# angelvillar96/STLPose

Hardware: AMD Instinct MI355X
Metric: images/sec/GPU HRNet-W32 384x288 train step; PCKh@0.5 parity (higher is better)
Workload: dtype f16/bf16; 1 GPU; HRNet-W32 384x288 bs=32/GPU train step (fwd+MSE+bwd+Adam), random-init weights; global_batch=32, parallelism=dp1

## Files before the change

### include/stlpose_hip.h

```cpp
#ifndef STLPOSE_HIP_H
#define STLPOSE_HIP_H
#include <stdint.h>
#ifdef __cplusplus
extern "C" {
#endif

#define STL_F32 0
#define STL_BF16 1
#define STL_F16 2
#define STL_NSHARD 2

#define STL_DT2(grad_dtype, fwd_dtype) ((grad_dtype) | ((fwd_dtype) << 8))

#define STL_SRC_PLAIN 0
#define STL_SRC_BN 1
#define STL_SRC_BNBWD 2
#define STL_SRC_BNADD 3

typedef struct stl_src {
    const void* x;
    const void* y;
    int32_t mode;
    int32_t relu;
    const double* stats;
// ... 16 lines not shown
    stl_src src;
    const void* w;
    void* out;
    const float* bias;
    int32_t out_relu;
    double* out_stats;
    const void* addend;
    const void* mask_y;
    stl_src mask_bn;
    double* red;
    const void* mask_z;
    void* src_out;
    int32_t ydtype, pad_;
} stl_conv;
int stl_conv_forward(const stl_conv* p, void* stream);
int stl_conv_plan(stl_conv* p);
int stl_conv_bnadd_ok(const stl_conv* p);

typedef struct stl_wgrad {
    int32_t dtype;
    int32_t B, Hi, Wi, Ci, Ho, Wo, Co, ks, stride;
    int32_t TH, TW, nsplit;
    stl_src h;
    stl_src g;
    float* partial;
    int32_t ydtype;
} stl_wgrad;
int stl_conv_wgrad(const stl_wgrad* p, void* stream);
#define STL_WGRAD_GROUP_MAX 8
typedef struct stl_wgrad_io { stl_src h; stl_src g; float* partial; } stl_wgrad_io;
typedef struct stl_wgrad_group { int32_t n, pad_; const stl_wgrad* p[STL_WGRAD_GROUP_MAX]; } stl_wgrad_group;
int stl_conv_wgrad_group(const stl_wgrad_group* g, void* stream);
int stl_wgrad_chunk(const stl_wgrad* p);

typedef struct stl_term {
    stl_src src;
    int32_t shift;
} stl_term;
typedef struct stl_fuse {
    int32_t dtype, B, H, W, C, nterms, relu;
    stl_term t[4];
    void* out;
} stl_fuse;
int stl_fuse_forward(const stl_fuse* p, void* stream);

typedef struct stl_fuse_bwd {
    int32_t dtype, B, H, W, C, ngrads, relu, nbn;
    const void* dz[4];
    const void* z;
    void* du;
    stl_src bn[4];
    double* rstats[4];
    int32_t ydtype, pad_;
} stl_fuse_bwd;
int stl_fuse_backward(const stl_fuse_bwd* p, void* stream);

typedef struct stl_upbwd {
    int32_t dtype, B, H, W, C, shift;
    const void* du;
    void* dt;
    stl_src bn;
    double* rstats;
    int32_t ydtype, pad_;
} stl_upbwd;
int stl_upsample_backward(const stl_upbwd* p, void* stream);

// ... 301 lines not shown
```

### stlpose_amd/build.py

```python
from __future__ import annotations

import glob
import hashlib
import os
import subprocess
import sys
from concurrent.futures import ThreadPoolExecutor

HERE = os.path.dirname(os.path.abspath(__file__))
CSRC = os.path.join(HERE, "csrc")
INCLUDE = os.path.join(HERE, "..", "include")
LIB = os.path.join(HERE, "libstlpose_hip.so")
UNITS = [("capi.hip", "capi", []), ("conv_core.hip", "conv_core_bf16", ["-DSTL_DT=1"]), ("conv_core.hip", "conv_core_f32", ["-DSTL_DT=0"]),
         ("conv_core.hip", "conv_core_f16", ["-DSTL_DT=3"]),
         ("wgrad.hip", "wgrad_bf16", ["-DSTL_DT=1"]), ("wgrad.hip", "wgrad_f32", ["-DSTL_DT=0"]), ("elementwise.hip", "elementwise", []),
         ("program.hip", "program", []), ("retrieval.hip", "retrieval", []),
         ("topdown.hip", "topdown", []), ("detector.hip", "detector", []), ("detector_train.hip", "detector_train", []),
         ("adain.hip", "adain", []), ("box_ap.hip", "box_ap", [])]
HIPCC = os.environ.get("HIPCC", "/opt/rocm/bin/hipcc")
FLAGS = ["--offload-arch=gfx950", "-O3", "-fPIC", "-std=c++17", "-Wno-unused-result", "-Wno-unused-value"]


def source_files():
    return sorted(glob.glob(os.path.join(CSRC, "*.hip")) + glob.glob(os.path.join(CSRC, "*.inc")) + glob.glob(os.path.join(CSRC, "*.cuh"))
                  + glob.glob(os.path.join(INCLUDE, "*.h")))


def source_id() -> str:
    h = hashlib.sha256()
    for f in source_files():
        h.update(os.path.basename(f).encode() + b"\0")
        h.update(open(f, "rb").read())
    return h.hexdigest()[:16]


def _digest(deps, flags) -> str:
    h = hashlib.sha256(" ".join(flags).encode())
    for f in deps:
        h.update(os.path.basename(f).encode() + b"\0")
        h.update(open(f, "rb").read())
    return h.hexdigest()[:16]


def _load_state(path: str) -> dict:
    try:
        import json
        return json.load(open(path))
    except Exception:
# ... 48 lines not shown
```

### stlpose_amd/capi.py

```python
from __future__ import annotations

import ctypes as C
import os

_HERE = os.path.dirname(os.path.abspath(__file__))
LIB_PATH = os.environ.get("STLPOSE_HIP_LIB") or os.path.join(_HERE, "libstlpose_hip.so")

F32, BF16, F16 = 0, 1, 2


def dt2(grad_dtype: int, fwd_dtype: int) -> int:
    return grad_dtype | ((fwd_dtype if fwd_dtype != grad_dtype else 0) << 8)


POSE_APPROACH = {"all_kpts": 0, "full_body": 1, "upper_body": 2}
POSE_DIM = {"all_kpts": 34, "full_body": 26, "upper_body": 18}
POSE_METHOD = {"euclidean": 0, "cosine": 1, "manhattan": 2, "confidence": 3, "oks": 4, "l2sq": 5, "cos_normalised": 6}
POSE_PEN = {"zero_coord": 0, "none": 1, "mean": 2, "max": 3}
POSE_TOPK_MAX, POSE_RANK_MAX, POSE_RANK_LABELS_MAX, POSE_NSCORES = 1024, 16384, 4, 10
POSE_RANK_ANY_MAX = 1 << 24
BOX_MAX, RESIZE_SRC_MAX, RESIZE_DST_MAX = 4096, 16384, 2048
BOX_AP_THRS, BOX_AP_AREAS, BOX_AP_DETS, BOX_AP_GT_MAX, BOX_AP_SCAN_TILE, BOX_AP_MAXDETS_MAX, BOX_AP_RECS_MAX = 10, 4, 100, 128, 1024, 8, 101
DET_NMS_MAX = 65536
GATHER_COPY, GATHER_UP, GATHER_POOL = 0, 1, 2
# ... 112 lines not shown

class DetTerm(C.Structure):
    _fields_ = [("x", vp), ("mode", i32), ("H", i32), ("W", i32), ("pad_", i32)]


class DetFuse(C.Structure):
    _fields_ = [("B", i32), ("H", i32), ("W", i32), ("C", i32), ("nterms", i32), ("pad_", i32), ("t", DetTerm * 3), ("wparam", vp),
                ("out", vp)]


class Op(C.Structure):
    _fields_ = [("kind", i32), ("stream", i32), ("desc", vp), ("nwait", i32), ("wait", i32 * 8), ("record", i32)]


class ReduceRange(C.Structure):
    _fields_ = [("partials", vp), ("grads", vp), ("tab", vp), ("n", i32), ("blk_base", i32), ("nblocks", i32), ("pad_", i32)]


class BNRange(C.Structure):
    _fields_ = [("rstats", vp), ("grads", vp), ("tab", vp), ("n", i32), ("pad_", i32)]


OP_KIND = {"stl_conv_forward": 0, "stl_conv_wgrad": 1, "stl_fuse_forward": 2, "stl_fuse_backward": 3,
           "stl_upsample_backward": 4, "stl_patch3x3": 5, "stl_head_forward": 6, "stl_head_backward": 7,
           "stl_reduce_slabs_range": 8, "stl_bn_grads_range": 9, "stl_conv_wgrad_group": 10,
           "stl_patch3x3_backward": 13}

SIGNATURES = {
    "stl_conv_forward": [C.POINTER(Conv), vp],
    "stl_conv_plan": [C.POINTER(Conv)],
    "stl_conv_bnadd_ok": [C.POINTER(Conv)],
    "stl_conv_wgrad": [C.POINTER(Wgrad), vp],
    "stl_wgrad_chunk": [C.POINTER(Wgrad)],
    "stl_conv_wgrad_group": [C.POINTER(WgradGroup), vp],
    "stl_fuse_forward": [C.POINTER(Fuse), vp],
    "stl_fuse_backward": [C.POINTER(FuseBwd), vp],
    "stl_upsample_backward": [C.POINTER(UpBwd), vp],
    "stl_patch3x3": [i32, vp, vp, i32, i32, i32, i32, vp, vp, vp],
    "stl_patch3x3_backward": [i32, vp, vp, i32, i32, i32, i32, vp, vp],
    "stl_head_forward": [i32, vp, vp, vp, vp, i32, i32, i32, i32, i32, vp],
    "stl_head_backward": [i32, vp, vp, vp, vp, vp, i32, i32, i32, i32, i32, i32, vp],
    "stl_mse_loss": [vp, vp, vp, vp, vp, i32, vp, i32, i32, i32, f32, vp],
    "stl_gaussian_targets": [vp, vp, vp, vp, i32, i32, i32, i32, f32, f32, f32, vp],
    "stl_heatmap_argmax": [vp, vp, vp, vp, i32, i32, i32, vp],
    "stl_flip_merge": [vp, vp, vp, vp, i32, i32, i32, i32, vp],
    "stl_flip_merge_backward": [vp, vp, vp, vp, i32, i32, i32, i32, vp],
    "stl_final_preds": [vp, vp, vp, vp, vp, i32, i32, i32, i32, vp],
    "stl_weight_prep": [i32, vp, vp, vp, i32, i32, vp],
    "stl_reduce_slabs": [vp, vp, vp, i32, i32, vp],
    "stl_reduce_slabs_range": [C.POINTER(ReduceRange), vp],
    "stl_bn_running_update": [vp, vp, vp, vp, i32, f32, vp, vp],
    "stl_bn_param_grads": [vp, vp, vp, i32, vp],
    "stl_adam_step": [vp, vp, vp, vp, i64, vp, vp, vp, vp],
    "stl_sgd_step": [vp, vp, vp, i64, vp, vp, vp, vp],
    "stl_affine_crop": [vp, vp, vp, vp, vp, vp, i32, i32, i32, vp, vp, vp],
    "stl_maxpool2x2": [i32, vp, vp, i32, i32, i32, i32, vp],
    "stl_l1_partial": [i32, vp, vp, i64, vp, i32, vp],
    "stl_l2_partial": [i32, vp, vp, i64, vp, i32, vp],
    "stl_maxpool2x2_backward": [i32, vp, vp, vp, i32, i32, i32, i32, i32, vp],
    "stl_l2_backward": [i32, vp, vp, vp, i64, vp, i32, vp],
    "stl_bilinear_nchw": [vp, vp, i32, i32, i32, i32, i32, i32, vp],
    "stl_sum_partials": [vp, i32, C.c_double, vp, i32, vp],
    "stl_nchw_to_nhwc": [i32, vp, vp, i32, i32, i32, i32, vp],
    "stl_nhwc_to_nchw": [i32, vp, vp, i32, i32, i32, i32, vp],
    "stl_program_create": [C.POINTER(Op), i32, i32, C.POINTER(vp)],
    "stl_program_run": [vp, C.POINTER(vp)],
# ... 95 lines not shown
```

### stlpose_amd/csrc/wgrad.hip

```cpp
#include <type_traits>
#include "common.cuh"

#ifndef STL_DT
#define STL_DT 2
#endif

constexpr int WG_MAXG = STL_WGRAD_GROUP_MAX;
struct WgK {
    stl_wgrad p;
    stl_wgrad_io io[WG_MAXG];
    int ng;
    int dbg;
    int tiles_c, npt, HR, HC, HP, PI, pad, taps;
    int psg, psh;
    int off_cg, off_ch, off_g, off_h;
    float r_TW, r_HC, r_tc, r_vp, r_PI;
    unsigned long long m_tc, m_vp, m_PI;
    int xmap, units, gy, gz;
};

int stl_wgrad_backend_bf16(bool wide, const WgK& k, dim3 grid, size_t lds, hipStream_t st);
int stl_wgrad_backend_f32(bool wide, const WgK& k, dim3 grid, size_t lds, hipStream_t st);

namespace {

#include "conv_common.inc"

#ifdef STL_STAMPS
#include "../../include/stlpose_hip_debug.h"
__device__ long long g_wstamps[16];
__device__ long long g_wstamps2[64];
#define WSTAMP(i)                                                                                   \
    do {                                                                                            \
        if (k.dbg && blockIdx.x == 0 && blockIdx.y == 0 && blockIdx.z == 0 && threadIdx.x == 0) g_wstamps[i] = wall_clock64(); \
    } while (0)
#define WSTAMP2(i)                                                                                  \
    do {                                                                                            \
        if (k.dbg && blockIdx.x == 0 && blockIdx.y == 0 && blockIdx.z == 0 && threadIdx.x == 0 && (i) < 64) g_wstamps2[i] = wall_clock64(); \
    } while (0)
#else
#define WSTAMP(i) do {} while (0)
#define WSTAMP2(i) do {} while (0)
#endif

__device__ __forceinline__ int mad24_vsv(int a, int b_uniform, int c) {
    int r;
    asm("v_mad_i32_i24 %0, %1, %2, %3" : "=v"(r) : "v"(a), "s"(b_uniform), "v"(c));
    return r;
}

__device__ __forceinline__ int sdiv(int n, unsigned long long m) { return (int)(((unsigned long long)(uint32_t)n * m) >> 32); }


struct WgBlock { int member, bsplit, cy, cz; bool live; };
__device__ __forceinline__ WgBlock wg_block(const WgK& k) {
// ... 563 lines not shown
#pragma unroll
        for (int mt = 0; mt < 2; ++mt)
#pragma unroll
            for (int nt = 0; nt < 2; ++nt) {
                const int co = co0 + wm * 32 + mt * 16 + 4 * g, ci = ci0 + wn * 32 + nt * 16 + (lane & 15);
                float* dst = slab + (size_t)co * TAPS * p.Ci + ci;
                const bool ciok = ci < p.Ci;
#pragma unroll
                for (int tap = 0; tap < TAPS; ++tap)
#pragma unroll
                    for (int r = 0; r < 4; ++r)
                        if (ciok && co + r < p.Co) dst[((size_t)r * TAPS + tap) * p.Ci] = acc[mt][nt][tap][r];
            }
    }
    WSTAMP(8);
}

template <typename T, typename TY, int KS, int NVH, bool GQ, int TPX>
int launch64(const WgK& k, dim3 grid, size_t lds, hipStream_t st) {
    static bool attr_done = false;
    if (!attr_done) {
        (void)hipFuncSetAttribute(reinterpret_cast<const void*>(&wgrad64_kernel<T, KS, NVH, GQ, TPX, TY>),
                                  hipFuncAttributeMaxDynamicSharedMemorySize, 160 * 1024);
        attr_done = true;
    }
    STL_LAUNCH((wgrad64_kernel<T, KS, NVH, GQ, TPX, TY>), grid, dim3(256), lds, st, k);
    static char nbuf[160];
    static const char* nm = stl_kname<T>(nbuf, "wgrad64_kernel", {KS, NVH, GQ, TPX, stl_code<TY>()});
    stl_note_kernel(nm, true);
    STL_LAUNCH_CHECK("conv_wgrad64");
    return 0;
}

#if STL_DT != 0
template <typename TY>
int dispatch64(const WgK& k, dim3 grid, size_t lds, hipStream_t st) {
    const int nvh = ceil_div(k.HP * 8, 256);
    const bool gq = k.p.g.mode == STL_SRC_BNBWD;
    if (k.p.TH * k.p.TW <= 128 && nvh <= 6) return gq ? launch64<__bf16, TY, 1, 6, true, 128>(k, grid, lds, st) : launch64<__bf16, TY, 1, 6, false, 128>(k, grid, lds, st);
    return stl_set_error("wgrad64: halo of %d pixels is too large for a %d-pixel tile", k.HP, k.p.TH * k.p.TW);
}
#endif

dim3 wg_grid(WgK& k, int units, int gy, int gz) {
    const int xcd_env = getenv("STL_WGRAD_XCD") ? atoi(getenv("STL_WGRAD_XCD")) : 1;
    k.units = units, k.gy = gy, k.gz = gz;
    k.xmap = xcd_env && gy * gz > 1;
    if (!k.xmap) return dim3(units, gy, gz);
    return dim3(8 * ceil_div(units, 8) * gy * gz, 1, 1);
}

static bool wgrad_c64_3x3(const stl_wgrad& p) {
    const char* e = getenv("STL_WGRAD_C64");
    return !(e && atoi(e) == 0) && p.dtype == STL_BF16 && p.ks == 3 && p.stride == 1 && p.Co >= 64 && p.Ci >= 64;
}

int wgrad_chunk(const stl_wgrad& p) {
    if (wgrad_c64_3x3(p)) return 64;
    return (p.dtype == STL_BF16 && p.ks == 1 && p.stride == 1 && p.Co >= 64 && p.Ci >= 64) ? 64 : 32;
}

template <typename T, typename TY, int KS>
int dispatch(const WgK& k, dim3 grid, size_t lds, hipStream_t st) {
    {
        const int64_t gpx = (int64_t)k.p.B * k.p.Ho * k.p.Wo, hpx = (int64_t)k.p.B * k.p.Hi * k.p.Wi;
        const bool small = gpx * k.p.Co * (int64_t)sizeof(T) < ((int64_t)1 << 32) && hpx * k.p.Ci * (int64_t)sizeof(T) < ((int64_t)1 << 32) &&
                           (int64_t)k.p.Wo * k.p.Co * (int64_t)sizeof(T) < (1 << 23) &&
                           (int64_t)(k.PI > k.p.Hi ? k.PI - k.p.Hi : k.p.Hi - k.PI) * k.p.Wi * k.p.Ci * (int64_t)sizeof(T) < (1 << 23) &&
                           k.PI < (1 << 12) && k.tiles_c < (1 << 12) && (int64_t)k.npt * k.p.TH * k.p.stride < (1 << 20);
        STL_CHECK(small, "wgrad: tensors of 4 GB or more, rows beyond 8 MB or more than 4095 rows / tile columns are not addressable");
    }
    const int vpx = 32 / ET<T>::KV;
    const int nvh = ceil_div(k.HP * vpx, 256);
    const bool gq = k.p.g.mode == STL_SRC_BNBWD;
    STL_CHECK(k.p.TH * k.p.TW <= 128, "wgrad: tiles of more than 128 pixels are not supported");
    if constexpr (KS == 3 && sizeof(T) == 2) {
        if (k.p.ks == 3 && wgrad_c64_3x3(k.p)) {
            const int nvh16 = ceil_div(k.HP * 8, 1024);
            if (nvh16 <= 2) return gq ? launch<T, TY, KS, 2, true, 128, 16, 64>(k, grid, lds, st) : launch<T, TY, KS, 2, false, 128, 16, 64>(k, grid, lds, st);
            if (nvh16 <= 3) return gq ? launch<T, TY, KS, 3, true, 128, 16, 64>(k, grid, lds, st) : launch<T, TY, KS, 3, false, 128, 16, 64>(k, grid, lds, st);
            return stl_set_error("wgrad: halo of %d pixels is too large for the 64-channel 3x3 kernel; shrink the tile", k.HP);
        }
    }
    if constexpr (KS == 3) {
        const int nvh8 = ceil_div(k.HP * vpx, 512);
        if (nvh8 <= 2) return gq ? launch<T, TY, KS, 2, true, 128, 8>(k, grid, lds, st) : launch<T, TY, KS, 2, false, 128, 8>(k, grid, lds, st);
        if (nvh8 <= 3) return gq ? launch<T, TY, KS, 3, true, 128, 8>(k, grid, lds, st) : launch<T, TY, KS, 3, false, 128, 8>(k, grid, lds, st);
        if (nvh8 <= 5) return gq ? launch<T, TY, KS, 5, true, 128, 8>(k, grid, lds, st) : launch<T, TY, KS, 5, false, 128, 8>(k, grid, lds, st);
        if (nvh8 <= 9) return gq ? launch<T, TY, KS, 9, true, 128, 8>(k, grid, lds, st) : launch<T, TY, KS, 9, false, 128, 8>(k, grid, lds, st);
        return stl_set_error("wgrad: halo of %d pixels is too large for the 3x3 kernel; shrink the tile", k.HP);
    }
    if (nvh <= 3) return gq ? launch<T, TY, KS, 3, true>(k, grid, lds, st) : launch<T, TY, KS, 3, false>(k, grid, lds, st);
    if (nvh <= 6) return gq ? launch<T, TY, KS, 6, true>(k, grid, lds, st) : launch<T, TY, KS, 6, false>(k, grid, lds, st);
    if (nvh <= 9) return gq ? launch<T, TY, KS, 9, true>(k, grid, lds, st) : launch<T, TY, KS, 9, false>(k, grid, lds, st);
    if (nvh <= 18) return gq ? launch<T, TY, KS, 18, true>(k, grid, lds, st) : launch<T, TY, KS, 18, false>(k, grid, lds, st);
    return stl_set_error("wgrad: halo of %d pixels needs %d staging vectors per thread (max 18); shrink the tile", k.HP, nvh);
}

}

#if STL_DT != 0
int stl_wgrad_backend_bf16(bool wide, const WgK& k, dim3 grid, size_t lds, hipStream_t st) {
    if (k.p.ydtype == STL_F16) {
        if (wide) return dispatch64<f16>(k, grid, lds, st);
        return k.p.ks == 3 ? dispatch<__bf16, f16, 3>(k, grid, lds, st) : dispatch<__bf16, f16, 1>(k, grid, lds, st);
    }
    if (wide) return dispatch64<__bf16>(k, grid, lds, st);
    return k.p.ks == 3 ? dispatch<__bf16, __bf16, 3>(k, grid, lds, st) : dispatch<__bf16, __bf16, 1>(k, grid, lds, st);
}
#endif
#if STL_DT != 1
int stl_wgrad_backend_f32(bool wide, const WgK& k, dim3 grid, size_t lds, hipStream_t st) {
    if (wide) return stl_set_error("wgrad: the 64 x 64-channel variant is bf16 only");
    return k.p.ks == 3 ? dispatch<float, float, 3>(k, grid, lds, st) : dispatch<float, float, 1>(k, grid, lds, st);
}
#endif

#if STL_DT != 0
#ifdef STL_STAMPS
extern "C" int stl_debug_wgrad_stamps2(long long* host64) {
    return hipMemcpyFromSymbol(host64, HIP_SYMBOL(g_wstamps2), 64 * sizeof(long long)) == hipSuccess ? 0 : stl_set_error("stamps: copy failed");
}
extern "C" int stl_debug_wgrad_stamps(long long* host16) {
    return hipMemcpyFromSymbol(host16, HIP_SYMBOL(g_wstamps), 16 * sizeof(long long)) == hipSuccess ? 0 : stl_set_error("stamps: copy failed");
}
#endif

extern "C" int stl_wgrad_chunk(const stl_wgrad* pp) { return wgrad_chunk(*pp); }

static int wgrad_run(const stl_wgrad* const* ps, int ng, void* stream);

extern "C" int stl_conv_wgrad(const stl_wgrad* pp, void* stream) { return wgrad_run(&pp, 1, stream); }

extern "C" int stl_conv_wgrad_group(const stl_wgrad_group* grp, void* stream) {
    STL_CHECK(grp && grp->n >= 1 && grp->n <= WG_MAXG, "wgrad_group: 1..%d members", WG_MAXG);
    const stl_wgrad& a = *grp->p[0];
    for (int i = 1; i < grp->n; ++i) {
        const stl_wgrad& b = *grp->p[i];
        STL_CHECK(b.dtype == a.dtype && b.B == a.B && b.Hi == a.Hi && b.Wi == a.Wi && b.Ci == a.Ci && b.Ho == a.Ho && b.Wo == a.Wo &&
                      b.Co == a.Co && b.ks == a.ks && b.stride == a.stride && b.TH == a.TH && b.TW == a.TW && b.nsplit == a.nsplit &&
                      b.g.mode == a.g.mode,
                  "wgrad_group: member %d differs from member 0 in geometry, tile, nsplit or gradient source mode", i);
    }
    return wgrad_run(grp->p, grp->n, stream);
}

static int wgrad_run(const stl_wgrad* const* ps, int ng, void* stream) {
    const stl_wgrad& p = *ps[0];
  for (int i_ = 0; i_ < ng; ++i_) {
    const stl_wgrad& p = *ps[i_];
    STL_CHECK(p.dtype == STL_F32 || p.dtype == STL_BF16, "wgrad: bad dtype (gradients are fp32 or bf16)");
    STL_CHECK(p.ydtype == 0 || p.ydtype == p.dtype || (p.dtype == STL_BF16 && p.ydtype == STL_F16), "wgrad: ydtype %d does not go with dtype %d", p.ydtype, p.dtype);
    STL_CHECK(p.ydtype == ps[0]->ydtype, "wgrad_group: members differ in ydtype");
    STL_CHECK(p.ks == 1 || p.ks == 3, "wgrad: ks must be 1 or 3");
    STL_CHECK(p.stride == 1 || p.stride == 2, "wgrad: stride must be 1 or 2");
    const int kv = p.dtype == STL_BF16 ? 8 : 4;
    STL_CHECK(p.Ci % kv == 0 && p.Co % kv == 0, "wgrad: Ci=%d / Co=%d must be multiples of %d", p.Ci, p.Co, kv);
    STL_CHECK(p.TH >= 1 && p.TW >= 1 && p.TH * p.TW <= 128, "wgrad: tile exceeds 128 pixels");
    STL_CHECK((int64_t)p.B * p.Hi * p.Wi * p.Ci < (1ll << 31) && (int64_t)p.B * p.Ho * p.Wo * p.Co < (1ll << 31),
              "wgrad: tensors of 2^31 or more elements are not supported");
    const int pad = p.ks == 3 ? 1 : 0;
    STL_CHECK((p.Hi + 2 * pad - p.ks) / p.stride + 1 == p.Ho && (p.Wi + 2 * pad - p.ks) / p.stride + 1 == p.Wo,
              "wgrad: output %dx%d inconsistent with input %dx%d", p.Ho, p.Wo, p.Hi, p.Wi);
    STL_CHECK(p.h.x && p.g.x && p.partial && p.nsplit >= 1, "wgrad: null pointer / nsplit");
    STL_CHECK(p.h.mode == STL_SRC_PLAIN || p.h.mode == STL_SRC_BN, "wgrad: h must be PLAIN or BN");
    STL_CHECK(p.g.mode == STL_SRC_PLAIN || p.g.mode == STL_SRC_BNBWD, "wgrad: g must be PLAIN or BNBWD");
    STL_CHECK(p.g.mode != STL_SRC_BNBWD || (p.g.y && p.g.stats && p.g.rstats && p.g.gamma), "wgrad: BNBWD source incomplete");
    STL_CHECK(p.h.mode != STL_SRC_BN || (p.h.gamma && p.h.beta && (p.h.stats || (p.h.rmean && p.h.rvar))), "wgrad: BN source incomplete");
  }
    const int pad = p.ks == 3 ? 1 : 0;
    WgK k;
    k.p = p;
    k.ng = ng;
    for (int i = 0; i < ng; ++i) k.io[i].h = ps[i]->h, k.io[i].g = ps[i]->g, k.io[i].partial = ps[i]->partial;
    k.dbg = getenv("STL_CONV_STAMPS") ? 1 : 0;
    k.taps = p.ks * p.ks;
    k.pad = pad;
    k.PI = p.stride * (p.Ho + 1);
    k.HR = (p.TH - 1) * p.stride + p.ks;
    k.HC = (p.TW - 1) * p.stride + p.ks;
    k.HP = k.HR * k.HC;
    k.tiles_c = ceil_div(p.Wo, p.TW);
    k.npt = ceil_div(p.B * (p.Ho + 1), p.TH) * k.tiles_c;
    k.r_TW = 1.0f / p.TW, k.r_HC = 1.0f / k.HC, k.r_tc = 1.0f / k.tiles_c, k.r_vp = 1.0f / (p.Ho + 1), k.r_PI = 1.0f / k.PI;
    const unsigned long long two32 = 1ull << 32;
    k.m_tc = (two32 + k.tiles_c - 1) / k.tiles_c, k.m_vp = (two32 + p.Ho) / (p.Ho + 1), k.m_PI = (two32 + k.PI - 1) / k.PI;
    STL_CHECK((int64_t)k.npt < (1 << 21) && (int64_t)p.B * k.PI < (1 << 21), "wgrad: too many tiles");
    hipStream_t st = (hipStream_t)stream;
    if (wgrad_c64_3x3(p)) {
        k.psg = k.psh = 64 * 2 + 32;
        k.off_cg = 0, k.off_ch = 3 * 64 * 4, k.off_g = 2048;
        k.off_h = k.off_g + 128 * k.psg;
        const size_t ldsw = (size_t)k.off_h + (size_t)k.HP * k.psh;
        STL_CHECK(ldsw <= 160 * 1024, "wgrad: tile needs %zu B of LDS (>160 KiB)", ldsw);
        STL_CHECK(p.nsplit <= k.npt || p.nsplit == 1, "wgrad: nsplit %d > tiles %d", p.nsplit, k.npt);
        dim3 gridw = wg_grid(k, p.nsplit * ng, ceil_div(p.Co, 64), ceil_div(p.Ci, 64));
        return stl_wgrad_backend_bf16(false, k, gridw, ldsw, st);
    }
    if (wgrad_chunk(p) == 64) {
        k.psg = k.psh = 160;
        k.off_cg = 0, k.off_ch = 3 * 64 * 4, k.off_g = 2048;
        k.off_h = k.off_g + 128 * k.psg;
        const size_t lds64 = (size_t)k.off_h + (size_t)k.HP * k.psh;
        STL_CHECK(lds64 <= 160 * 1024, "wgrad64: tile needs %zu B of LDS (>160 KiB)", lds64);
        STL_CHECK(p.nsplit <= k.npt || p.nsplit == 1, "wgrad: nsplit %d > tiles %d", p.nsplit, k.npt);
        dim3 grid64 = wg_grid(k, p.nsplit * ng, ceil_div(p.Co, 64), ceil_div(p.Ci, 64));
        return stl_wgrad_backend_bf16(true, k, grid64, lds64, st);
    }
    const int esz = p.dtype == STL_BF16 ? 2 : 4;
    k.psg = k.psh = 32 * esz + (esz == 2 ? 32 : 16);
    k.off_cg = 0;
    k.off_ch = 3 * 32 * 4;
    k.off_g = 1024;
    int szG = 128 * k.psg;
    int szH = k.HP * k.psh;
    k.off_h = k.off_g + szG;
    size_t lds = (size_t)k.off_h + szH;
    STL_CHECK(lds <= 160 * 1024, "wgrad: tile needs %zu B of LDS (>160 KiB)", lds);
    STL_CHECK(p.nsplit <= k.npt || p.nsplit == 1, "wgrad: nsplit %d > tiles %d", p.nsplit, k.npt);
    dim3 grid = wg_grid(k, p.nsplit * ng, ceil_div(p.Co, 32), ceil_div(p.Ci, 32));
    return p.dtype == STL_BF16 ? stl_wgrad_backend_bf16(false, k, grid, lds, st) : stl_wgrad_backend_f32(false, k, grid, lds, st);
// ... 3 lines not shown
```

### stlpose_amd/engine.py

```python
from __future__ import annotations

import bisect
import ctypes as C
import math
import os
from dataclasses import dataclass, field
from typing import Dict, List, NamedTuple, Optional, Tuple, Union

import torch

from . import capi
from .arch import Arch, Registry, registry, walk

EPS = 1e-5
MOMENTUM = 0.1


def _esz(dtype: int) -> int:
    return 4 if (dtype & 0xff) == capi.F32 else 2


def choose_tile(B: int, Ho: int, Wo: int, stride: int, ks: int, esz: int, bn_cols: int = 64,
                maxpx: int = 128, maxhalo: int = 576) -> Tuple[int, int]:
    vrows = B * (Ho + 1)
# ... 162 lines not shown
        self.dtype, self.fdtype = dtype & 0xff, ((dtype >> 8) & 0xff) or (dtype & 0xff)
        self.ydtype = self.fdtype if self.fdtype != self.dtype else 0
        self.training = training
        self.input_grad = input_grad
        self.dev = store.device
        self.esz = _esz(dtype)
        self.tdtype = torch.float32 if self.dtype == capi.F32 else torch.bfloat16
        self.lib = capi.lib()
        self.fwd_ops: List[Launch] = []
        self.bwd_ops: List[Launch] = []
        self.tape: List[Union[ConvNode, FuseNode, HeadNode]] = []
        self.convs: List[ConvInfo] = []
        self.bns: List[BNInfo] = []
        self._keep: List = []
        self._progs: Dict[str, C.c_void_p] = {}
        self._fixups: Dict[str, List[Tuple]] = {}
        self.act_bytes = 0
        self.generation = 0
        self.img = torch.zeros(B, 3, H, W, dtype=torch.float32, device=self.dev)
        self.out: Optional[torch.Tensor] = None
        self.dout: Optional[torch.Tensor] = None
        self.dimg: Optional[torch.Tensor] = None
        nstat = bn_stat_elems(store.reg)
        self.stats = torch.zeros(max(nstat, 1), dtype=torch.float64, device=self.dev)
        self.rstats = torch.zeros(max(nstat, 1), dtype=torch.float64, device=self.dev) if training or input_grad else None
        self.sink = torch.zeros(max(nstat, 1), dtype=torch.float64, device=self.dev) if input_grad and not training else None
        self.overflow = torch.full((1,), 2 ** 31 - 1, dtype=torch.int32, device=self.dev)
        env = os.environ.get
        self.nstreams = int(env("STLPOSE_STREAMS", "4"))
        self.merge_minc = int(env("STLPOSE_MERGE_MINC", "128"))
        self.bucket_mb = float(env("STLPOSE_BUCKET_MB", "64"))
        self.wgrad_blocks = int(env("STLPOSE_WGRAD_BLOCKS", "256" if self.esz == 2 else "512"))
        self.wgrad_blocks_wide = int(env("STLPOSE_WGRAD_BLOCKS_WIDE", str(self.wgrad_blocks // 2)))
        self.wgrad_group = int(env("STLPOSE_WGRAD_GROUP", "4"))
        self.wgrad_group_wide = int(env("STLPOSE_WGRAD_GROUP_WIDE", "8"))
        self._poison = env("STLPOSE_POISON", "0") != "0"
        self._stream = 0
        self._side = None
        self._stats_used = 0
        self._wk_elems = 0
        walk(self, arch)
        self._check_stats_arena(nstat)
        self._finalize_weights()
        self._build_tables()
        if training or input_grad:
            self._build_backward()
        assert not self._fixups, "descriptor fields left pointing into arenas that were never allocated"

    def _check_stats_arena(self, nstat: int):
        if self._stats_used != nstat:
            raise RuntimeError(f"engine: the plan uses {self._stats_used} statistics elements, the arenas hold {nstat}")

    def _alloc(self, nbytes: int) -> torch.Tensor:
        self.act_bytes += nbytes
        t = torch.empty(nbytes, dtype=torch.uint8, device=self.dev)
        if self._poison:
            t.fill_(0xFF)
        self._keep.append(t)
        return t

    def _act_tensor(self, B, H, W, C) -> torch.Tensor:
        return self._alloc(B * H * W * C * self.esz)

    def _fix(self, desc, attr: str, arena: str, off: int):
        self._fixups.setdefault(arena, []).append((desc, attr, off))

# ... 307 lines not shown
    def _add_slab(self, part_off, grad_off, nsplit, Co, Ci, ks, Cip, patch, stride=0):
        self.slabs.append(capi.Slab(part_off, grad_off, nsplit, Co, Ci, ks, Cip, patch, self._slab_blocks, stride))
        self._slab_blocks += math.ceil(Co * Ci * ks * ks / 1024)

    def _bucket_close(self, force: bool = False):
        bk, st = self._bucket, self.store
        complete = bk.done == bk.hi - bk.lo
        force = force or (complete and bk.lo in {st.param_off.get(k) for k in ("transition1.0.0.weight", "layer1.1.conv1.weight")})
        if not complete or bk.done == 0 or (bk.done < int(self.bucket_mb * (1 << 20) / 4) and not force):
            return
        for key in list(self._wg_pending):
            self._flush_wgrad_group(key)
        grads = st.grads.data_ptr()
        blk0 = self.slabs[bk.slab0].blk0
        rr = capi.ReduceRange(grads=grads, n=len(self.slabs) - bk.slab0, blk_base=blk0, nblocks=self._slab_blocks - blk0)
        self._fix(rr, "partials", "slab", 0)
        self._fix(rr, "tab", "slab_tab", bk.slab0 * C.sizeof(capi.Slab))
        i0, i1 = bisect.bisect_left(self._bn_offs, bk.lo), bisect.bisect_left(self._bn_offs, bk.hi)
        br = capi.BNRange(rstats=self.rstats.data_ptr(), grads=grads, tab=self._bn_tab.data_ptr() + i0 * C.sizeof(capi.BNRec),
                          n=i1 - i0)
        self._emit("stl_reduce_slabs_range", rr, bk.stream, bk.reads, [C.addressof(rr)])
        self._emit("stl_bn_grads_range", br, bk.stream, [C.addressof(rr)], [C.addressof(br)])
        self.buckets.append(Bucket(bk.lo, bk.hi, len(self.bwd_ops) - 1))
        bk.hi, bk.done, bk.slab0, bk.reads = bk.lo, 0, len(self.slabs), []

    def _op_cost_us(self, name: str, d) -> float:
        esz = self.esz
        if name == "stl_conv_forward":
            src = d.B * d.Hi * d.Wi * d.Ci * (2 if d.src.mode == capi.SRC_BNBWD else 1)
            out = d.B * d.Ho * d.Wo * d.Co * (1 + bool(d.mask_y) + bool(d.addend) + bool(d.mask_z))
            return 12.0 + (src + out) * esz / 2.0e6
        if name == "stl_conv_wgrad":
            by = (d.B * d.Hi * d.Wi * d.Ci + d.B * d.Ho * d.Wo * d.Co * (2 if d.g.mode == capi.SRC_BNBWD else 1)) * esz
            return 16.0 + (by + 2.0 * d.nsplit * d.Co * d.Ci * d.ks * d.ks * 4) / 2.0e6
        if name == "stl_conv_wgrad_group":
            m = d.members[0]
            by = (m.B * m.Hi * m.Wi * m.Ci + m.B * m.Ho * m.Wo * m.Co * (2 if m.g.mode == capi.SRC_BNBWD else 1)) * esz
            return 16.0 + d.n * (by + 2.0 * m.nsplit * m.Co * m.Ci * m.ks * m.ks * 4) / 2.0e6
        if name == "stl_fuse_backward":
            return 8.0 + d.B * d.H * d.W * d.C * (d.ngrads + 2 + d.nbn) * esz / 3.0e6
        if name == "stl_upsample_backward":
            return 8.0 + d.B * d.H * d.W * d.C * ((1 << (2 * d.shift)) + 2) * esz / 3.0e6
        if name == "stl_head_backward":
            return 80.0
        if name == "stl_reduce_slabs_range":
            return 20.0 + 80.0 * d.nblocks / 1100.0
        return 5.0

    def _emit(self, name: str, desc, stream: int, reads: list, writes: list):
        acc = self.sched_estimate_us
        if name in ("stl_conv_wgrad", "stl_conv_wgrad_group", "stl_reduce_slabs_range", "stl_bn_grads_range"):
            own = stream % self.nstreams
            cands = list(range(self._active, self.nstreams)) + [own]
            if self._active == 1:
                cands = list(range(1, min(3, self.nstreams))) + [own]
            stream = min(cands, key=lambda s_: (acc[s_], s_ != own))
        acc[stream] += self._op_cost_us(name, desc)
        self.bwd_ops.append(Launch(name, desc, stream, reads, writes))

    def _emit_wgrad(self, n: ConvNode, g: capi.Src):
        x, y, ci, kks, kstride = n.x, n.y, n.conv, n.ks, n.stride
        wg = capi.Wgrad()
        wg.dtype, wg.ydtype = self.dtype, self.ydtype
        wg.B, wg.Hi, wg.Wi, wg.Ci, wg.Ho, wg.Wo, wg.Co = x.B, x.H, x.W, x.C, y.H, y.W, y.C
        wg.ks, wg.stride = kks, kstride
        ctile = capi.lib().stl_wgrad_chunk(C.byref(wg))
        wide3 = ctile == 64 and kks == 3
        wg.TH, wg.TW = choose_tile(x.B, y.H, y.W, kstride, kks, self.esz, bn_cols=32, maxhalo=(256 if wide3 else 192) if ctile == 64 else 576)
        npt = math.ceil(x.B * (y.H + 1) / wg.TH) * math.ceil(y.W / wg.TW)
        chunks = math.ceil(y.C / ctile) * math.ceil(x.C / ctile)
        budget = self.wgrad_blocks_wide if wide3 else self.wgrad_blocks
        tail = self._active_of(ci.key) == 1
        gmax = self.wgrad_group_wide if wide3 else self.wgrad_group
        gsize = 1 if tail else max(1, min(gmax, capi.WGRAD_GROUP_MAX, max(1, budget // chunks)))
        bg = budget // gsize
        top = max(1, min(npt, bg // chunks if chunks <= bg else 1))
        wg.nsplit = min(range(1, top + 1), key=lambda ns: (math.ceil(npt / ns) + 0.004 * ns * chunks / 8, ns))
        wg.h = self._src(x)
        wg.g = g
        part_off = self._slab_alloc(wg, wg.nsplit * y.C * kks * kks * x.C)
        self._add_slab(part_off, ci.master_off, wg.nsplit, ci.Co, ci.Ci, ci.ks, ci.Cik, int(ci.patch))
        self._bucket.reads.append(C.addressof(wg))
        self._bucket.stream = n.stream
        key = (x.C, y.C, kks, kstride, x.H, x.W, wg.TH, wg.TW, wg.nsplit, int(g.mode), gsize)
        pend = self._wg_pending.setdefault(key, [])
        pend.append(Launch("stl_conv_wgrad", wg, n.stream, [y.dt.data_ptr(), x.ptr], [C.addressof(wg)]))
        if len(pend) >= gsize:
            self._flush_wgrad_group(key)

    def _flush_wgrad_group(self, key):
        pend = self._wg_pending.pop(key)
        if len(pend) == 1:
            self._emit(*pend[0])
            return
        members = [op.desc for op in pend]
        grp = capi.WgradGroup()
        grp.n = len(members)
        for i, wg in enumerate(members):
            grp.p[i] = C.pointer(wg)
        grp.members = members
        self._emit("stl_conv_wgrad_group", grp, pend[-1].stream, [r for op in pend for r in op.reads],
                   [w for op in pend for w in op.writes])

    def _build_tables(self):
        tab = [capi.BNRec(b.stats_off, b.param_off, b.buf_off, b.C, b.inv_count) for b in self.bns]
        self._bn_tab = _to_device((capi.BNRec * len(tab))(*tab), self.dev)
        assert len(self.bns) == self.store.nnbt
        self._bn_offs = [b.param_off for b in self.bns]
        assert self._bn_offs == sorted(self._bn_offs)

# ... 91 lines not shown
        if self.training and update_running:
            st = self.store
            capi.call("stl_bn_running_update", self.stats.data_ptr(), st.bufs.data_ptr(), st.nbt.data_ptr(),
                      self._bn_tab.data_ptr(), len(self.bns), MOMENTUM, self.overflow.data_ptr(), stream)

    NO_OVERFLOW = 2 ** 31 - 1

    def check_forward_range(self):
        i = int(self.overflow.item())
        if i == self.NO_OVERFLOW:
            return
        self.overflow.fill_(self.NO_OVERFLOW)
        bn = self.bns[i]
        name = next((k for k, off in self.store.param_off.items() if off == bn.param_off), f"BatchNorm #{i}")
        what = {capi.F16: "f16 (|y| > 65504)", capi.BF16: "bf16", capi.F32: "fp32"}[self.fdtype]
        raise FloatingPointError(
            f"stlpose_amd: the raw output of the convolution in front of {name[:-len('.weight')] if name.endswith('.weight') else name} "
            f"left the range of its {what} storage (non-finite BatchNorm statistics; first such layer in forward order).  "
            "The optimiser skipped that step (and skips every step until this is reported): the weights are intact; the running "
            "statistics of the layers behind it took their momentum update from the poisoned pass.  Forward tensors of the default "
            "'mixed' mode are f16; for a checkpoint with badly scaled weights use compute_dtype='bf16' (same speed, bf16 range) "
            "or 'fp32'.")

    def backward(self, stream: int, on_bucket=None):
        assert self.training or self.input_grad
        if self.training:
            self.rstats.zero_()
        self._run(self._program("bwd"), stream, on_bucket if self.buckets else None)

    def bucket_wait(self, i: int, stream: int):
        capi.call("stl_program_wait_op", self._program("bwd"), self.buckets[i].op, stream)


_STREAM_POOL: Dict[int, Dict] = {}


def bn_weight_keys(reg: Registry) -> set:
    return {k[: -len("running_mean")] + "weight" for k, _ in reg.buffers if k.endswith("running_mean")}


def bn_stat_elems(reg: Registry) -> int:
    keys = bn_weight_keys(reg)
    return sum(int(math.prod(s)) for k, s in reg.params if k in keys) * 2 * capi.NSHARD


def _to_device(ctab, device) -> torch.Tensor:
    raw = bytes(ctab)
    t = torch.frombuffer(bytearray(raw), dtype=torch.uint8).clone()
    return t.to(device)
```

Measured before the change: 2444 images/sec.

## Add streaming single-block-per-slab 1x1 wgrad kernel with adaptive nsplit

Adds a new 1x1 stride-1 bf16 weight-gradient kernel. One 512-thread block covers the whole Co x Ci output (up to 16384 elements) and streams pixel tiles through double-buffered registers and LDS, so no channel-chunk grid is needed. The engine now asks the library how many channel chunks a layer needs, marks such layers as streaming, and for tail layers chooses nsplit with a cost model that weighs tile traffic against partial-slab traffic. This is meant to stop re-reading the activations once per channel chunk for small-channel 1x1 convs. The cost is a new compiled unit, heavier register and LDS use per block, and possibly lower occupancy.

```diff
diff --git a/include/stlpose_hip.h b/include/stlpose_hip.h
--- a/include/stlpose_hip.h
+++ b/include/stlpose_hip.h
@@ -72,6 +72,7 @@
 typedef struct stl_wgrad_group { int32_t n, pad_; const stl_wgrad* p[STL_WGRAD_GROUP_MAX]; } stl_wgrad_group;
 int stl_conv_wgrad_group(const stl_wgrad_group* g, void* stream);
 int stl_wgrad_chunk(const stl_wgrad* p);
+int stl_wgrad_chunk_blocks(const stl_wgrad* p);
 
 typedef struct stl_term {
     stl_src src;
diff --git a/stlpose_amd/build.py b/stlpose_amd/build.py
--- a/stlpose_amd/build.py
+++ b/stlpose_amd/build.py
@@ -13,7 +13,8 @@
 LIB = os.path.join(HERE, "libstlpose_hip.so")
 UNITS = [("capi.hip", "capi", []), ("conv_core.hip", "conv_core_bf16", ["-DSTL_DT=1"]), ("conv_core.hip", "conv_core_f32", ["-DSTL_DT=0"]),
          ("conv_core.hip", "conv_core_f16", ["-DSTL_DT=3"]),
-         ("wgrad.hip", "wgrad_bf16", ["-DSTL_DT=1"]), ("wgrad.hip", "wgrad_f32", ["-DSTL_DT=0"]), ("elementwise.hip", "elementwise", []),
+         ("wgrad.hip", "wgrad_bf16", ["-DSTL_DT=1"]), ("wgrad.hip", "wgrad_f32", ["-DSTL_DT=0"]),
+         ("wgrad.hip", "wgrad_stream", ["-DSTL_DT=4"]), ("elementwise.hip", "elementwise", []),
          ("program.hip", "program", []), ("retrieval.hip", "retrieval", []),
          ("topdown.hip", "topdown", []), ("detector.hip", "detector", []), ("detector_train.hip", "detector_train", []),
          ("adain.hip", "adain", []), ("box_ap.hip", "box_ap", [])]
diff --git a/stlpose_amd/capi.py b/stlpose_amd/capi.py
--- a/stlpose_amd/capi.py
+++ b/stlpose_amd/capi.py
@@ -168,6 +168,7 @@
     "stl_conv_bnadd_ok": [C.POINTER(Conv)],
     "stl_conv_wgrad": [C.POINTER(Wgrad), vp],
     "stl_wgrad_chunk": [C.POINTER(Wgrad)],
+    "stl_wgrad_chunk_blocks": [C.POINTER(Wgrad)],
     "stl_conv_wgrad_group": [C.POINTER(WgradGroup), vp],
     "stl_fuse_forward": [C.POINTER(Fuse), vp],
     "stl_fuse_backward": [C.POINTER(FuseBwd), vp],
diff --git a/stlpose_amd/csrc/wgrad.hip b/stlpose_amd/csrc/wgrad.hip
--- a/stlpose_amd/csrc/wgrad.hip
+++ b/stlpose_amd/csrc/wgrad.hip
@@ -4,6 +4,9 @@
 #ifndef STL_DT
 #define STL_DT 2
 #endif
+#define STL_WG_BF16 (STL_DT == 1 || STL_DT == 2)
+#define STL_WG_F32 (STL_DT == 0 || STL_DT == 2)
+#define STL_WG_STREAM (STL_DT == 4 || STL_DT == 2)
 
 constexpr int WG_MAXG = STL_WGRAD_GROUP_MAX;
 struct WgK {
@@ -21,6 +24,7 @@
 
 int stl_wgrad_backend_bf16(bool wide, const WgK& k, dim3 grid, size_t lds, hipStream_t st);
 int stl_wgrad_backend_f32(bool wide, const WgK& k, dim3 grid, size_t lds, hipStream_t st);
+int stl_wgrad_backend_stream(int layout, const WgK& k, dim3 grid, hipStream_t st);
 
 namespace {
 
@@ -650,7 +654,11 @@
     return 0;
 }
 
-#if STL_DT != 0
+#if STL_WG_STREAM
+#include "wgrad_stream.inc"
+#endif
+
+#if STL_WG_BF16
 template <typename TY>
 int dispatch64(const WgK& k, dim3 grid, size_t lds, hipStream_t st) {
     const int nvh = ceil_div(k.HP * 8, 256);
@@ -676,6 +684,19 @@
 int wgrad_chunk(const stl_wgrad& p) {
     if (wgrad_c64_3x3(p)) return 64;
     return (p.dtype == STL_BF16 && p.ks == 1 && p.stride == 1 && p.Co >= 64 && p.Ci >= 64) ? 64 : 32;
+}
+
+[[maybe_unused]] static int wg_stream_layout(const stl_wgrad& p) {
+    const char* e = getenv("STL_WGRAD_1X1_STREAM");
+    if (e && atoi(e) == 0) return -1;
+    if (p.dtype != STL_BF16 || p.ks != 1 || p.stride != 1 || p.Co < 32 || p.Ci < 32 || (int64_t)p.Co * p.Ci > 16384) return -1;
+    const int big = p.Co > p.Ci ? p.Co : p.Ci;
+    if (p.Ho + 1 >= (1 << 12) || p.Wo >= (1 << 12) || (int64_t)p.B * (p.Ho + 1) >= (1 << 19) || (int64_t)p.Wo * big * 2 >= (1 << 23)) return -1;
+    const int cot = ceil_div(p.Co, 16), cit = ceil_div(p.Ci, 16);
+    static const int lay[5][2] = {{4, 4}, {16, 4}, {4, 16}, {16, 5}, {12, 8}};
+    for (int i = 0; i < 5; ++i)
+        if (cot <= lay[i][0] && cit <= lay[i][1]) return i;
+    return -1;
 }
 
 template <typename T, typename TY, int KS>
@@ -717,7 +738,13 @@
 
 }
 
-#if STL_DT != 0
+#if STL_WG_STREAM
+int stl_wgrad_backend_stream(int layout, const WgK& k, dim3 grid, hipStream_t st) {
+    return k.p.ydtype == STL_F16 ? dispatch_stream<f16>(layout, k, grid, st) : dispatch_stream<__bf16>(layout, k, grid, st);
+}
+#endif
+
+#if STL_WG_BF16
 int stl_wgrad_backend_bf16(bool wide, const WgK& k, dim3 grid, size_t lds, hipStream_t st) {
     if (k.p.ydtype == STL_F16) {
         if (wide) return dispatch64<f16>(k, grid, lds, st);
@@ -727,14 +754,14 @@
     return k.p.ks == 3 ? dispatch<__bf16, __bf16, 3>(k, grid, lds, st) : dispatch<__bf16, __bf16, 1>(k, grid, lds, st);
 }
 #endif
-#if STL_DT != 1
+#if STL_WG_F32
 int stl_wgrad_backend_f32(bool wide, const WgK& k, dim3 grid, size_t lds, hipStream_t st) {
     if (wide) return stl_set_error("wgrad: the 64 x 64-channel variant is bf16 only");
     return k.p.ks == 3 ? dispatch<float, float, 3>(k, grid, lds, st) : dispatch<float, float, 1>(k, grid, lds, st);
 }
 #endif
 
-#if STL_DT != 0
+#if STL_WG_BF16
 #ifdef STL_STAMPS
 extern "C" int stl_debug_wgrad_stamps2(long long* host64) {
     return hipMemcpyFromSymbol(host64, HIP_SYMBOL(g_wstamps2), 64 * sizeof(long long)) == hipSuccess ? 0 : stl_set_error("stamps: copy failed");
@@ -745,6 +772,12 @@
 #endif
 
 extern "C" int stl_wgrad_chunk(const stl_wgrad* pp) { return wgrad_chunk(*pp); }
+
+extern "C" int stl_wgrad_chunk_blocks(const stl_wgrad* pp) {
+    if (wg_stream_layout(*pp) >= 0) return 1;
+    const int c = wgrad_chunk(*pp);
+    return ceil_div(pp->Co, c) * ceil_div(pp->Ci, c);
+}
 
 static int wgrad_run(const stl_wgrad* const* ps, int ng, void* stream);
 
@@ -805,6 +838,13 @@
     k.m_tc = (two32 + k.tiles_c - 1) / k.tiles_c, k.m_vp = (two32 + p.Ho) / (p.Ho + 1), k.m_PI = (two32 + k.PI - 1) / k.PI;
     STL_CHECK((int64_t)k.npt < (1 << 21) && (int64_t)p.B * k.PI < (1 << 21), "wgrad: too many tiles");
     hipStream_t st = (hipStream_t)stream;
+    if (const int layout = wg_stream_layout(p); layout >= 0) {
+        STL_CHECK(p.nsplit <= k.npt || p.nsplit == 1, "wgrad: nsplit %d > tiles %d", p.nsplit, k.npt);
+        STL_CHECK((int64_t)k.npt * p.TH < (1 << 20) && k.tiles_c < (1 << 12), "wgrad stream: too many tiles");
+        k.psg = k.psh = 0, k.off_cg = k.off_ch = k.off_g = k.off_h = 0;
+        dim3 grids = wg_grid(k, p.nsplit * ng, 1, 1);
+        return stl_wgrad_backend_stream(layout, k, grids, st);
+    }
     if (wgrad_c64_3x3(p)) {
         k.psg = k.psh = 64 * 2 + 32;
         k.off_cg = 0, k.off_ch = 3 * 64 * 4, k.off_g = 2048;
diff --git a/stlpose_amd/csrc/wgrad_stream.inc b/stlpose_amd/csrc/wgrad_stream.inc
--- /dev/null
+++ b/stlpose_amd/csrc/wgrad_stream.inc
@@ -0,0 +1,245 @@
+template <int WM, int MA, int NB>
+struct WgStreamCfg {
+    static constexpr int WN = 8 / WM;
+    static constexpr int COT = WM * MA, CIT = WN * NB;
+    static constexpr int CGP = COT * 16, CHP = CIT * 16;
+    static constexpr int PSG = COT * 32 + (COT % 2 ? 64 : 32), PSH = CIT * 32 + (CIT % 2 ? 64 : 32);
+    static constexpr int OFF_CG = 0, OFF_CH = 3 * CGP * 4;
+    static constexpr int OFF_G = (OFF_CH + 2 * CHP * 4 + 255) / 256 * 256;
+    static constexpr int OFF_H = OFF_G + 128 * PSG;
+    static constexpr int LDS = OFF_H + 128 * PSH;
+    static_assert(WM * WN == 8 && CGP <= 256 && CHP <= 256 && MA * NB * 4 <= 64, "wave grid / constants / accumulators");
+    static_assert((PSG / 32) % 2 == 1 && (PSH / 32) % 2 == 1 && 3 * 32 * PSG + COT * 32 < 65536 && 3 * 32 * PSH + CIT * 32 < 65536, "LDS strides");
+    static_assert(LDS <= 160 * 1024, "LDS");
+};
+
+template <typename TY, bool GQ, int WM, int MA, int NB, int NSET>
+__global__ __launch_bounds__(512, 1) void wgrad1x1_stream_kernel(const WgK k) {
+    using T = __bf16;
+    using CF = WgStreamCfg<WM, MA, NB>;
+    extern __shared__ __attribute__((aligned(16))) char smem[];
+    constexpr int KV = 8, KSTEP = 32, NR = 2, TPX = 128, NT = 512, NKT = TPX / KSTEP;
+    constexpr int VG = 2 * CF::COT, VH = 2 * CF::CIT;
+    constexpr int NVG = (TPX * VG + NT - 1) / NT, NVH = (TPX * VH + NT - 1) / NT;
+    constexpr int PSG = CF::PSG, PSH = CF::PSH;
+    const stl_wgrad& p = k.p;
+    const WgBlock wb = wg_block(k);
+    if (!wb.live) return;
+    const int bsplit = wb.bsplit;
+    const stl_wgrad_io& io = k.io[wb.member];
+    const int tid = threadIdx.x, lane = tid & 63, wave = tid >> 6, g = lane >> 4;
+    const int wm = wave / CF::WN, wn = wave % CF::WN;
+    float* cgc = reinterpret_cast<float*>(smem + CF::OFF_CG);
+    float* chc = reinterpret_cast<float*>(smem + CF::OFF_CH);
+    char* sG = smem + CF::OFF_G;
+    char* sH = smem + CF::OFF_H;
+
+    const int tilepx = p.TH * p.TW;
+    const int vpitch = p.Ho + 1;
+    const int nks = (tilepx + KSTEP - 1) / KSTEP;
+
+    const int g_cbytes = p.Co * (int)sizeof(T), h_cbytes = p.Ci * (int)sizeof(T);
+    const int g_wrap = -p.Wo * g_cbytes, h_wrap = -p.Wo * h_cbytes;
+    const int n_vp = -vpitch;
+    const int g_rbytes = p.Wo * g_cbytes, h_rbytes = p.Wo * h_cbytes;
+
+    V16 rgv[NSET][NVG], rgq[NSET][GQ ? NVG : 1], rhv[NSET][NVH];
+    uint32_t okm[NSET] = {};
+
+    auto tile_offsets = [&](int t, uint32_t* go, uint32_t* ho) __attribute__((always_inline)) -> uint32_t {
+        const int tr = sdiv(t, k.m_tc), tc = t - tr * k.tiles_c;
+        const int vr0 = tr * p.TH, c0 = tc * p.TW;
+        const int gb0 = sdiv(vr0, k.m_vp), gy0 = vr0 - gb0 * vpitch;
+        const int px0 = (vr0 - gb0) * p.Wo + c0;
+        const uint32_t g_t = (uint32_t)(px0 * g_cbytes), h_t = (uint32_t)(px0 * h_cbytes);
+        uint32_t ok = 0;
+#pragma unroll
+        for (int i = 0; i < NVG; ++i) {
+            const int v = tid + i * NT, m = v / VG, part = v % VG;
+            const int ty = fdiv(m, k.r_TW), tx = m - ty * p.TW;
+            const int oy0 = gy0 + ty, c = c0 + tx;
+            const int wr_ = fdiv(oy0, k.r_vp);
+            const int oy = mad24_vsv(wr_, n_vp, oy0);
+            const bool in = (m < tilepx) & (part * KV < p.Co) & (gb0 + wr_ < p.B) & (oy < p.Ho) & (c < p.Wo);
+            const int lo = mad24_vsv(ty, g_rbytes, mad24_vsv(tx, g_cbytes, (int)g_t + part * 16));
+            const uint32_t off = (uint32_t)mad24_vsv(wr_, g_wrap, lo);
+            go[i] = in ? off : 0u;
+            asm("" : "+v"(go[i]));
+            ok |= in ? 1u << i : 0u;
+        }
+#pragma unroll
+        for (int i = 0; i < NVH; ++i) {
+            const int v = tid + i * NT, m = v / VH, part = v % VH;
+            const int ty = fdiv(m, k.r_TW), tx = m - ty * p.TW;
+            const int oy0 = gy0 + ty, c = c0 + tx;
+            const int wr_ = fdiv(oy0, k.r_vp);
+            const int oy = mad24_vsv(wr_, n_vp, oy0);
+            const bool in = (m < tilepx) & (part * KV < p.Ci) & (gb0 + wr_ < p.B) & (oy < p.Ho) & (c < p.Wo);
+            const int lo = mad24_vsv(ty, h_rbytes, mad24_vsv(tx, h_cbytes, (int)h_t + part * 16));
+            const uint32_t off = (uint32_t)mad24_vsv(wr_, h_wrap, lo);
+            ho[i] = in ? off : 0u;
+            asm("" : "+v"(ho[i]));
+            ok |= in ? 1u << (NVG + i) : 0u;
+        }
+        return ok;
+    };
+    auto fetch = [&](auto SET, int t) __attribute__((always_inline)) {
+        constexpr int S = decltype(SET)::value;
+        uint32_t go[NVG], ho[NVH];
+        const uint32_t ok = tile_offsets(t, go, ho);
+#pragma unroll
+        for (int i = 0; i < NVG; ++i) {
+            rgv[S][i] = ldg16((const char*)io.g.x + go[i]);
+            if (GQ) rgq[S][i] = ldg16((const char*)io.g.y + go[i]);
+        }
+#pragma unroll
+        for (int i = 0; i < NVH; ++i) rhv[S][i] = ldg16((const char*)io.h.x + ho[i]);
+        okm[S] = ok;
+        __builtin_amdgcn_sched_barrier(0);
+    };
+    const float relu_lo = io.h.relu ? 0.f : -INFINITY;
+    auto write_lds = [&](auto SET) __attribute__((always_inline)) {
+        constexpr int S = decltype(SET)::value;
+#pragma unroll
+        for (int i = 0; i < NVG; ++i) {
+            const int v = tid + i * NT, cl = (v % VG) * KV;
+            V16 val = rgv[S][i];
+            if (GQ) val = xform_bnbwd<T, TY>(val, rgq[S][i], cgc + cl, cgc + CF::CGP + cl, cgc + 2 * CF::CGP + cl);
+            mask16(val, (okm[S] >> i) & 1u);
+            if ((i + 1) * NT <= TPX * VG || v < TPX * VG) *reinterpret_cast<V16*>(sG + (v / VG) * PSG + (v % VG) * 16) = val;
+            if (GQ) __builtin_amdgcn_sched_barrier(0);
+        }
+#pragma unroll
+        for (int i = 0; i < NVH; ++i) {
+            const int v = tid + i * NT, cl = (v % VH) * KV;
+            V16 val = rhv[S][i];
+            if (io.h.mode == STL_SRC_BN) val = xform_bn<T, TY>(val, chc + cl, chc + CF::CHP + cl, relu_lo);
+            else val = xform_cvt<T, TY>(val);
+            mask16(val, (okm[S] >> (NVG + i)) & 1u);
+            if ((i + 1) * NT <= TPX * VH || v < TPX * VH) *reinterpret_cast<V16*>(sH + (v / VH) * PSH + (v % VH) * 16) = val;
+        }
+    };
+
+    f32x4 acc[MA][NB];
+#pragma unroll
+    for (int a = 0; a < MA; ++a)
+#pragma unroll
+        for (int b = 0; b < NB; ++b) acc[a][b] = f32x4{0.f, 0.f, 0.f, 0.f};
+
+    uint32_t gaw[NR], hbw[NR];
+#pragma unroll
+    for (int i = 0; i < NR; ++i) {
+        const int c = krow16(g, i, lane);
+        gaw[i] = (uint32_t)(uintptr_t)sG + c * PSG + (lane & 3) * 8 + wm * MA * 32;
+        hbw[i] = (uint32_t)(uintptr_t)sH + c * PSH + (lane & 3) * 8 + wn * NB * 32;
+    }
+    auto mfma_tile = [&]() __attribute__((always_inline)) {
+        uint32_t ga[NR], hb[NR];
+#pragma unroll
+        for (int i = 0; i < NR; ++i) {
+            ga[i] = gaw[i], hb[i] = hbw[i];
+            asm volatile("" : "+v"(ga[i]));
+            asm volatile("" : "+v"(hb[i]));
+        }
+#pragma unroll
+        for (int s = 0; s < NKT; ++s) {
+            if (s < nks) {
+                V16 af[MA], bf[NB];
+#pragma unroll
+                for (int a = 0; a < MA; ++a) af[a] = frag_at<T>(ga, s * KSTEP * PSG + a * 32);
+#pragma unroll
+                for (int b = 0; b < NB; ++b) bf[b] = frag_at<T>(hb, s * KSTEP * PSH + b * 32);
+#pragma unroll
+                for (int b = 0; b < NB; ++b)
+#pragma unroll
+                    for (int a = 0; a < MA; ++a) mma16<T>(acc[a][b], af[a], bf[b]);
+            }
+        }
+    };
+
+    const int step = p.nsplit;
+    int t = bsplit;
+    SrcRaw raw;
+    const bool cg = tid < 256;
+    const int cch = cg ? tid : tid - 256;
+    const bool cw = cg ? cch < CF::CGP : cch < CF::CHP;
+    const bool cok = cw && (cg ? cch < p.Co : cch < p.Ci);
+    if (cok) {
+        if (cg) src_raw_load(io.g, cch, p.Co, raw);
+        else src_raw_load(io.h, cch, p.Ci, raw);
+    }
+    constexpr std::integral_constant<int, 0> I0{};
+    constexpr std::integral_constant<int, 1> I1{};
+    fetch(I0, t);
+    if constexpr (NSET == 2) fetch(I1, t + step);
+    if (cw) {
+        float a = 0.f, b = 0.f, cc = 0.f;
+        if (cok) {
+            if (cg) src_raw_finish(io.g, raw, a, b, cc);
+            else src_raw_finish(io.h, raw, a, b, cc);
+        }
+        if (cg) cgc[cch] = a, cgc[CF::CGP + cch] = b, cgc[2 * CF::CGP + cch] = cc;
+        else chc[cch] = a, chc[CF::CHP + cch] = b;
+    }
+    __syncthreads();
+    auto body = [&](auto SET) __attribute__((always_inline)) {
+        const bool live = t < k.npt;
+        if (live) write_lds(SET);
+        __syncthreads();
+        fetch(SET, t + NSET * step);
+        if (live) mfma_tile();
+        __syncthreads();
+        t += step;
+    };
+    while (t < k.npt) {
+        body(I0);
+        if constexpr (NSET == 2) body(I1);
+    }
+    {
+        float* slab = io.partial + (size_t)bsplit * p.Co * p.Ci;
+#pragma unroll
+        for (int a = 0; a < MA; ++a)
+#pragma unroll
+            for (int b = 0; b < NB; ++b) {
+                const int co = (wm * MA + a) * 16 + 4 * g, ci = (wn * NB + b) * 16 + (lane & 15);
+                float* dst = slab + (size_t)co * p.Ci + ci;
+#pragma unroll
+                for (int r = 0; r < 4; ++r)
+                    if (ci < p.Ci && co + r < p.Co) dst[(size_t)r * p.Ci] = acc[a][b][r];
+            }
+    }
+}
+
+template <typename TY, bool GQ, int WM, int MA, int NB, int NSET>
+int launch_stream(const WgK& k, dim3 grid, hipStream_t st) {
+    using CF = WgStreamCfg<WM, MA, NB>;
+    static bool attr_done = false;
+    if (!attr_done) {
+        (void)hipFuncSetAttribute(reinterpret_cast<const void*>(&wgrad1x1_stream_kernel<TY, GQ, WM, MA, NB, NSET>),
+                                  hipFuncAttributeMaxDynamicSharedMemorySize, 160 * 1024);
+        attr_done = true;
+    }
+    STL_LAUNCH((wgrad1x1_stream_kernel<TY, GQ, WM, MA, NB, NSET>), grid, dim3(512), (size_t)CF::LDS, st, k);
+    static char nbuf[160];
+    static const char* nm = stl_kname<__bf16>(nbuf, "wgrad1x1_stream_kernel", {GQ, WM, MA, NB, NSET, stl_code<TY>()});
+    stl_note_kernel(nm, true);
+    STL_LAUNCH_CHECK("conv_wgrad_stream");
+    return 0;
+}
+
+template <typename TY, int WM, int MA, int NB, int NSET = 2>
+int launch_stream_gq(const WgK& k, dim3 grid, hipStream_t st) {
+    return k.p.g.mode == STL_SRC_BNBWD ? launch_stream<TY, true, WM, MA, NB, NSET>(k, grid, st) : launch_stream<TY, false, WM, MA, NB, NSET>(k, grid, st);
+}
+
+template <typename TY>
+int dispatch_stream(int layout, const WgK& k, dim3 grid, hipStream_t st) {
+    switch (layout) {
+    case 0: return launch_stream_gq<TY, 4, 1, 2>(k, grid, st);
+    case 1: return launch_stream_gq<TY, 8, 2, 4>(k, grid, st);
+    case 2: return launch_stream_gq<TY, 1, 4, 2>(k, grid, st);
+    case 3: return launch_stream_gq<TY, 8, 2, 5, 1>(k, grid, st);
+    case 4: return launch_stream_gq<TY, 4, 3, 4, 1>(k, grid, st);
+    }
+    return stl_set_error("wgrad stream: no layout %d", layout);
+}
diff --git a/stlpose_amd/engine.py b/stlpose_amd/engine.py
--- a/stlpose_amd/engine.py
+++ b/stlpose_amd/engine.py
@@ -218,6 +218,8 @@
         self.bucket_mb = float(env("STLPOSE_BUCKET_MB", "64"))
         self.wgrad_blocks = int(env("STLPOSE_WGRAD_BLOCKS", "256" if self.esz == 2 else "512"))
         self.wgrad_blocks_wide = int(env("STLPOSE_WGRAD_BLOCKS_WIDE", str(self.wgrad_blocks // 2)))
+        self.wgrad_stream = env("STL_WGRAD_1X1_STREAM", "1") != "0"
+        self.wgrad_blocks_stream = int(env("STLPOSE_WGRAD_BLOCKS_STREAM", "128"))
         self.wgrad_group = int(env("STLPOSE_WGRAD_GROUP", "4"))
         self.wgrad_group_wide = int(env("STLPOSE_WGRAD_GROUP_WIDE", "8"))
         self._poison = env("STLPOSE_POISON", "0") != "0"
@@ -591,7 +593,8 @@
             return 12.0 + (src + out) * esz / 2.0e6
         if name == "stl_conv_wgrad":
             by = (d.B * d.Hi * d.Wi * d.Ci + d.B * d.Ho * d.Wo * d.Co * (2 if d.g.mode == capi.SRC_BNBWD else 1)) * esz
-            return 16.0 + (by + 2.0 * d.nsplit * d.Co * d.Ci * d.ks * d.ks * 4) / 2.0e6
+            rate = STREAM_WGRAD_BYTES_PER_US if getattr(d, "streaming", False) else 2.0e6
+            return 16.0 + (by + 2.0 * d.nsplit * d.Co * d.Ci * d.ks * d.ks * 4) / rate
         if name == "stl_conv_wgrad_group":
             m = d.members[0]
             by = (m.B * m.Hi * m.Wi * m.Ci + m.B * m.Ho * m.Wo * m.Co * (2 if m.g.mode == capi.SRC_BNBWD else 1)) * esz
@@ -627,14 +630,22 @@
         wide3 = ctile == 64 and kks == 3
         wg.TH, wg.TW = choose_tile(x.B, y.H, y.W, kstride, kks, self.esz, bn_cols=32, maxhalo=(256 if wide3 else 192) if ctile == 64 else 576)
         npt = math.ceil(x.B * (y.H + 1) / wg.TH) * math.ceil(y.W / wg.TW)
-        chunks = math.ceil(y.C / ctile) * math.ceil(x.C / ctile)
+        chunks = capi.lib().stl_wgrad_chunk_blocks(C.byref(wg))
+        wg.streaming = (self.wgrad_stream and chunks == 1 and kks == 1 and kstride == 1 and self.dtype == capi.BF16
+                        and x.C >= 32 and y.C >= 32)
         budget = self.wgrad_blocks_wide if wide3 else self.wgrad_blocks
         tail = self._active_of(ci.key) == 1
         gmax = self.wgrad_group_wide if wide3 else self.wgrad_group
         gsize = 1 if tail else max(1, min(gmax, capi.WGRAD_GROUP_MAX, max(1, budget // chunks)))
         bg = budget // gsize
         top = max(1, min(npt, bg // chunks if chunks <= bg else 1))
-        wg.nsplit = min(range(1, top + 1), key=lambda ns: (math.ceil(npt / ns) + 0.004 * ns * chunks / 8, ns))
+        if wg.streaming and tail:
+            top = max(1, min(npt, self.wgrad_blocks_stream))
+            tile_by = wg.TH * wg.TW * (x.C + y.C * (2 if g.mode == capi.SRC_BNBWD else 1)) * self.esz
+            slab_by = y.C * x.C * 4
+            wg.nsplit = min(range(1, top + 1), key=lambda ns: (math.ceil(npt / ns) * top * tile_by + 2.33 * ns * slab_by, ns))
+        else:
+            wg.nsplit = min(range(1, top + 1), key=lambda ns: (math.ceil(npt / ns) + 0.004 * ns * chunks / 8, ns))
         wg.h = self._src(x)
         wg.g = g
         part_off = self._slab_alloc(wg, wg.nsplit * y.C * kks * kks * x.C)
@@ -792,6 +803,8 @@
         capi.call("stl_program_wait_op", self._program("bwd"), self.buckets[i].op, stream)
 
 
+STREAM_WGRAD_BYTES_PER_US = 3.5e6
+
 _STREAM_POOL: Dict[int, Dict] = {}
 
 
```

Result: no change. 2440 images/sec (-0.2%).
